# bentherien/point-cloud-reid

Measured on AMD Instinct MI355X. Metric: siamese pair-comparisons/sec @1024 pts, higher is better.
Workload: dtype bf16x3

## Files before the change

point-cloud-reid_amd/csrc/attn_kernels_impl.h:

```cpp
#pragma once
#ifndef PCR_ATTN_PREC
#define PCR_ATTN_PREC 0
#endif
#include "tile_dense.h"

#include <stdio.h>

#include <vector>

namespace {
constexpr int kAPrec = PCR_ATTN_PREC;
struct AttnArgs {
  pcr_attn_params p;
  int dbg;
};

constexpr int kATraceWgs = 512, kATraceRecs = 24, kATraceMarks = 8;
__device__ unsigned long long g_attn_trace[2 * kATraceWgs * kATraceRecs * kATraceMarks];


__device__ __forceinline__ void pos_hidden(float *dst, int RP, const float *P, const float *w0,
                                           const float *b0, int d, int T) {
  for (int e = threadIdx.x; e < d * T; e += blockDim.x) {
    const int o = e / T, t = e - o * T;
    const float v = w0[o * 3] * P[t] + w0[o * 3 + 1] * P[RP + t] + w0[o * 3 + 2] * P[2 * RP + t] + b0[o];
    dst[o * RP + t] = fmaxf(v, 0.f);
  }
}

__device__ __forceinline__ void load_xyz3(float *P, int RP, const float *xyz, int L, int t0, int T) {
  for (int e = threadIdx.x; e < 3 * T; e += blockDim.x) {
    const int c = e / T, t = e - c * T;
    P[c * RP + t] = t0 + t < L ? xyz[(size_t)(t0 + t) * 3 + c] : 0.f;
  }
}

__device__ __forceinline__ void attn_kv_fold_write(const pcr_attn_params &p, const float *KVl, const float *s_kt, size_t b) {
  const int d = p.d, dh = d / p.nhead, ld = d + 1, tid = threadIdx.x;
  float *kv = p.kv + b * ((size_t)d * d + d);
  const int d_o = kThreads / d, d_dd = kThreads - d_o * d;
  int o = tid / d, dd = tid - o * d;
  int v0 = (dd / dh) * dh;
  for (int e = tid; e < d * d; e += kThreads, o += d_o, dd += d_dd) {
    if (dd >= d) {
      dd -= d;
      o++;
    }
    if (d_dd) v0 = (dd / dh) * dh;
    const float *wm = p.wmerge + (size_t)o * d + v0;
    const float *kr = KVl + dd * ld + v0;
    float m = 0.f;
#pragma unroll 8
    for (int v = 0; v < dh; v++) m += wm[v] * kr[v];
    if constexpr (kAPrec == 0) {
      const int kb = dd >> 3, rem = dd & 7;
      kv[(((size_t)kb * d + o) * 2 + (rem & 1)) * 4 + (rem >> 1)] = m;
    } else {
      const int s16 = dd >> 4, kk = dd & 15;
      const int hh = (kk >> 2) & 1, jj = (kk & 3) + ((kk >> 3) << 2);
      const size_t unit = (((size_t)s16 * (d >> 5) + (o >> 5)) * 2) * 64 + hh * 32 + (o & 31);
      const __bf16 hi = (__bf16)m;
      const __bf16 lo = (__bf16)(m - (float)hi);
      __bf16 *img = reinterpret_cast<__bf16 *>(kv);
      img[unit * 8 + jj] = hi;
      img[(unit + 64) * 8 + jj] = lo;
    }
  }
  __syncthreads();
  if (tid < d) kv[(size_t)d * d + tid] = s_kt[tid];
}

__device__ __forceinline__ void attn_kv_fold_mfma(const pcr_attn_params &p, const float *KVt, const float *s_kt, size_t b) {
  const int d = p.d, dh = d / p.nhead, ld = d + 1, tid = threadIdx.x;
  float *kv = p.kv + b * ((size_t)d * d + d);
  for (int hd = 0; hd < p.nhead; hd++) {
    const float *wm = p.wmerge_packed + (size_t)(hd * dh / 8) * d * 8;
    tile_dense(KVt + (size_t)(hd * dh) * ld + hd * dh, dh, ld, dh >> 5, wm, d, [&](float m, int o, int t) {
      const int dd = hd * dh + t;
      if constexpr (kAPrec == 0) {
        const int kb = dd >> 3, rem = dd & 7;
        kv[(((size_t)kb * d + o) * 2 + (rem & 1)) * 4 + (rem >> 1)] = m;
      } else {
        const int s16 = dd >> 4, kk = dd & 15;
        const int hh = (kk >> 2) & 1, jj = (kk & 3) + ((kk >> 3) << 2);
        const size_t unit = (((size_t)s16 * (d >> 5) + (o >> 5)) * 2) * 64 + hh * 32 + (o & 31);
        const __bf16 hi = (__bf16)m;
        const __bf16 lo = (__bf16)(m - (float)hi);
        __bf16 *img = reinterpret_cast<__bf16 *>(kv);
        img[unit * 8 + jj] = hi;
        img[(unit + 64) * 8 + jj] = lo;
      }
    });
  }
  __syncthreads();
  if (tid < d) kv[(size_t)d * d + tid] = s_kt[tid];
}

// ... 1200 lines not shown
          const float tm = up ? vm[r + N] : vm[r], um = up ? vm[r] : vm[r + N];                       \
          const float ts = up ? vs[r + N] : vs[r], us = up ? vs[r] : vs[r + N];                       \
          vm[r] = fmaxf(tm, __uint_as_float(pcr_sort_partner<2 * J, J>(__float_as_uint(um), lane)));  \
          vs[r] = ts + __uint_as_float(pcr_sort_partner<2 * J, J>(__float_as_uint(us), lane));        \
        }                                                                                             \
      }
      PCR_POOL_STEP(8, 2, 2)
      PCR_POOL_STEP(4, 4, 4)
      PCR_POOL_STEP(2, 8, 8)
      PCR_POOL_STEP(1, 16, 16)
#undef PCR_POOL_STEP
      pmax = fmaxf(pmax, vm[0]);
      psum += vs[0];
      if (++pblk == nblk) {
        const int e = ((j & 1) << 4) | ((j & 2) << 2) | (j & 4) | ((j & 8) >> 2) | ((j & 16) >> 4);
        const int ch = 16 * (e >> 3) + bf_kpos(h, e & 7);
        float *po = p.pool_out + (size_t)b * 128;
        po[ch] = pmax;
        po[64 + ch] = psum;
        pmax = -INFINITY;
        psum = 0.f;
        pblk = 0;
        pc += nwav;
      }
    } else if constexpr (!CF) {
      const __amdgpu_buffer_rsrc_t rout =
          __builtin_amdgcn_make_buffer_rsrc(p.out + (size_t)b * (32 * NOB) * p.Lq, 0, 32 * NOB * p.Lq * 4, 0x00020000);
#pragma unroll
      for (int e = 0; e < 16 * NOB; e++) {
        const int ch = 16 * (e >> 3) + bf_kpos(0, e & 7);
        const float v = o[e >> 4][e & 15];
        __builtin_amdgcn_raw_buffer_store_b32(__builtin_bit_cast(unsigned, v), rout, vo, ch * p.Lq * 4, 0);
      }
    } else {
#pragma unroll
      for (int cb = 0; cb < NOB; cb++)
#pragma unroll
        for (int G = 0; G < 2; G++) to_ops(o[cb], G, bh[2 * cb + G], bl[2 * cb + G]);
      f32x16 fo[CF ? CF : 1];
#pragma unroll
      for (int cb = 0; cb < CF; cb++)
#pragma unroll
        for (int r = 0; r < 16; r++) fo[cb][r] = 0.f;
      const bf16x8 *wb = reinterpret_cast<const bf16x8 *>(p.wfinal) + lane;
#pragma unroll
      for (int s2 = 0; s2 < 2 * NOB; s2++) {
        bf16x8 wh[CF ? CF : 1], wl[CF ? CF : 1];
#pragma unroll
        for (int cb = 0; cb < CF; cb++) {
          wh[cb] = wb[((s2 * CF + cb) * 2) * 64];
          wl[cb] = wb[((s2 * CF + cb) * 2 + 1) * 64];
        }
#pragma unroll
        for (int cb = 0; cb < CF; cb++) fo[cb] = __builtin_amdgcn_mfma_f32_32x32x16_bf16(wh[cb], bh[s2], fo[cb], 0, 0, 0);
#pragma unroll
        for (int cb = 0; cb < CF; cb++) fo[cb] = __builtin_amdgcn_mfma_f32_32x32x16_bf16(wh[cb], bl[s2], fo[cb], 0, 0, 0);
#pragma unroll
        for (int cb = 0; cb < CF; cb++) fo[cb] = __builtin_amdgcn_mfma_f32_32x32x16_bf16(wl[cb], bh[s2], fo[cb], 0, 0, 0);
      }
      const __amdgpu_buffer_rsrc_t rout =
          __builtin_amdgcn_make_buffer_rsrc(p.out + (size_t)b * (32 * CF) * p.Lq, 0, 32 * CF * p.Lq * 4, 0x00020000);
#pragma unroll
      for (int cb = 0; cb < CF; cb++)
#pragma unroll
        for (int g = 0; g < 4; g++) {
          const f32x4 bv = cvec(s_c + 320, cb, g);
#pragma unroll
          for (int qq = 0; qq < 4; qq++) {
            const int e = 16 * cb + 4 * g + qq;
            const int ch = 16 * (e >> 3) + bf_kpos(0, e & 7);
            const float v = fo[cb][4 * g + qq] + bv[qq];
            __builtin_amdgcn_raw_buffer_store_b32(__builtin_bit_cast(unsigned, v), rout, vo, ch * p.Lq * 4, 0);
          }
        }
    }
    __builtin_amdgcn_wave_barrier();
    PCR_AMARK(7);
    PCR_ANEXT();
  }
#undef PCR_AMARK
#undef PCR_ANEXT
}

template <int NB>
__device__ __forceinline__ void ap128_step(f32x16 (&acc)[NB], const bf16x8 *wb, int ls, const bf16x8 &bh, const bf16x8 &bl) {
#pragma unroll
  for (int c0 = 0; c0 < NB; c0 += 4) {
    bf16x8 wh[4], wl[4];
#pragma unroll
    for (int cb = 0; cb < 4; cb++) {
      wh[cb] = wb[((ls * NB + c0 + cb) * 2) * 64];
      wl[cb] = wb[((ls * NB + c0 + cb) * 2 + 1) * 64];
    }
#pragma unroll
    for (int cb = 0; cb < 4; cb++) acc[c0 + cb] = __builtin_amdgcn_mfma_f32_32x32x16_bf16(wh[cb], bh, acc[c0 + cb], 0, 0, 0);
#pragma unroll
    for (int cb = 0; cb < 4; cb++) acc[c0 + cb] = __builtin_amdgcn_mfma_f32_32x32x16_bf16(wh[cb], bl, acc[c0 + cb], 0, 0, 0);
#pragma unroll
    for (int cb = 0; cb < 4; cb++) acc[c0 + cb] = __builtin_amdgcn_mfma_f32_32x32x16_bf16(wl[cb], bh, acc[c0 + cb], 0, 0, 0);
    asm volatile("" ::: "memory");
  }
}
constexpr int kAp128Waves = 4, kAp128ChunkU = 2048, kAp128Chunks = 16;
constexpr size_t kAp128Lds = (size_t)2 * kAp128ChunkU * 16 + (640 + 4 * 128 + kAp128Waves * 128) * sizeof(float);
template <int NH>
__global__ __launch_bounds__(64 * kAp128Waves) __attribute__((amdgpu_waves_per_eu(1, 1)))
void attn_apply_stream128_kernel(AttnArgs a) {
  constexpr int D = 128, ND = 4, SD = 8, GPH = 8 / NH;
  constexpr int NPC = kAp128ChunkU / (64 * kAp128Waves);
  extern __shared__ __attribute__((aligned(16))) float smem[];
  const pcr_attn_params &p = a.p;
  f32x4 *s_ring = reinterpret_cast<f32x4 *>(smem);
  int coff = 2 * kAp128ChunkU * 4;
  asm volatile("" : "+s"(coff));
  float *s_c = smem + coff;
  f32x4 *s_p0 = reinterpret_cast<f32x4 *>(s_c + 640);
  float *s_ks = s_c + 640 + 4 * 128;
  const int tid = threadIdx.x, lane = tid & 63, j = lane & 31, h = lane >> 5;
  const int wave = __builtin_amdgcn_readfirstlane(tid >> 6);
  const __amdgpu_buffer_rsrc_t rwq = __builtin_amdgcn_make_buffer_rsrc(const_cast<float *>(p.wq), 0, 4 * kAp128ChunkU * 16, 0x00020000),
                               rw0 = __builtin_amdgcn_make_buffer_rsrc(const_cast<float *>(p.wmlp0), 0, 8 * kAp128ChunkU * 16, 0x00020000),
                               rw2 = __builtin_amdgcn_make_buffer_rsrc(const_cast<float *>(p.wmlp2), 0, 4 * kAp128ChunkU * 16, 0x00020000);
  f32x4 stg[NPC];
  auto fetch = [&](int k) __attribute__((always_inline)) {
    k %= kAp128Chunks;
    const __amdgpu_buffer_rsrc_t r = k < 4 ? rwq : (k < 12 ? rw0 : rw2);
    const int kk = k < 4 ? k : (k < 12 ? k - 4 : k - 12);
#pragma unroll
    for (int u = 0; u < NPC; u++)
      stg[u] = __builtin_bit_cast(f32x4, __builtin_amdgcn_raw_buffer_load_b128(r, tid * 16, (kk * kAp128ChunkU + u * 64 * kAp128Waves) * 16, 0));
    asm volatile("" ::: "memory");
  };
  auto commit = [&](int k) __attribute__((always_inline)) {
    f32x4 *dst = s_ring + (k & 1) * kAp128ChunkU + tid;
#pragma unroll
    for (int u = 0; u < NPC; u++) dst[u * 64 * kAp128Waves] = stg[u];
    __syncthreads();
  };
  for (int e = tid; e < D; e += 64 * kAp128Waves) {
    s_c[e] = p.bq[e];
    s_c[128 + e] = p.ln1_g[e];
    s_c[256 + e] = p.ln1_b[e];
    s_c[384 + e] = p.ln2_g[e];
    s_c[512 + e] = p.ln2_b[e];
    s_p0[e] = f32x4{p.pos0_w[3 * e], p.pos0_w[3 * e + 1], p.pos0_w[3 * e + 2], p.pos0_b[e]};
  }
  fetch(0);
  commit(0);
  const int nblk = p.Lq >> 5;
  const long nitem = (long)p.B * nblk;
  const float skf = (float)p.Sk;
  float *ksw = s_ks + wave * 128;
  auto cvec = [&](const float *base, int cb, int g) __attribute__((always_inline)) {
    return *reinterpret_cast<const f32x4 *>(base + 32 * cb + 8 * g + 4 * h);
  };
  auto to_ops = [&](const f32x16 &acc, int G, bf16x8 &oh, bf16x8 &ol) __attribute__((always_inline)) {
    float v[8];
#pragma unroll
    for (int e = 0; e < 8; e++) v[e] = acc[8 * G + e];
    bf_split8(v, oh, ol, true);
  };
  auto layernorm = [&](f32x16 (&v)[ND], const float *gam, const float *bet) __attribute__((always_inline)) {
    float sm = 0.f;
#pragma unroll
    for (int cb = 0; cb < ND; cb++)
#pragma unroll
      for (int r = 0; r < 16; r++) sm += v[cb][r];
    sm += __shfl_xor(sm, 32, 64);
    const float mean = sm / (float)D;
    float vr = 0.f;
#pragma unroll
    for (int cb = 0; cb < ND; cb++)
#pragma unroll
      for (int r = 0; r < 16; r++) {
        const float dlt = v[cb][r] - mean;
        vr += dlt * dlt;
      }
    vr += __shfl_xor(vr, 32, 64);
    const float inv = 1.0f / sqrtf(vr / (float)D + 1e-5f);
#pragma unroll
    for (int cb = 0; cb < ND; cb++)
#pragma unroll
      for (int g = 0; g < 4; g++) {
        const f32x4 gv = cvec(gam, cb, g), bv = cvec(bet, cb, g);
#pragma unroll
        for (int qq = 0; qq < 4; qq++) v[cb][4 * g + qq] = (v[cb][4 * g + qq] - mean) * inv * gv[qq] + bv[qq];
      }
  };
  for (long it0 = (long)blockIdx.x * kAp128Waves; it0 < nitem; it0 += (long)gridDim.x * kAp128Waves) {
    const long item = it0 + wave;
    const bool live = item < nitem;
    const long it = live ? item : nitem - 1;
    const long b = it / nblk;
    const int blk = (int)(it - b * nblk);
    const size_t bq_ = p.q_index ? (size_t)p.q_index[b] : (size_t)b;
    const size_t kb_ = p.kv_index ? (size_t)p.kv_index[b] : (size_t)b;
    const float *kvp = p.kv + kb_ * ((size_t)D * D + D);
    const int t = blk * 32 + j;
    const __amdgpu_buffer_rsrc_t rfeat = __builtin_amdgcn_make_buffer_rsrc(
        const_cast<float *>(p.feat_q + bq_ * D * p.Lq), 0, D * p.Lq * 4, 0x00020000);
    const int vo = (4 * h * p.Lq + t) * 4;
    auto load_x = [&](float (&xf)[64]) __attribute__((always_inline)) {
#pragma unroll
      for (int e = 0; e < 64; e++) {
        const int ch = 16 * (e >> 3) + bf_kpos(0, e & 7);
        xf[e] = __builtin_bit_cast(float, __builtin_amdgcn_raw_buffer_load_b32(rfeat, vo, ch * p.Lq * 4, 0));
      }
    };
    ksw[lane] = kvp[(size_t)D * D + lane];
    ksw[64 + lane] = kvp[(size_t)D * D + 64 + lane];
    bf16x8 bh[16], bl[16];
    {
      float xf[64];
      load_x(xf);
      const float *xyz = p.xyz_q + (bq_ * p.Lq + t) * 3;
      const float px = xyz[0], py = xyz[1], pz = xyz[2];
#pragma unroll
      for (int s2 = 0; s2 < SD; s2++) {
        float hv[8];
#pragma unroll
        for (int e = 0; e < 8; e++) {
// ... 70 lines not shown
#pragma unroll
        for (int r = 0; r < 16; r++) q[cb][r] = 0.f;
      const bf16x8 *mb = reinterpret_cast<const bf16x8 *>(kvp) + lane;
      bf16x8 mh[2][ND], ml[2][ND];
#pragma unroll
      for (int cb = 0; cb < ND; cb++) {
        mh[0][cb] = mb[(cb * 2) * 64];
        ml[0][cb] = mb[(cb * 2 + 1) * 64];
      }
#pragma unroll
      for (int s2 = 0; s2 < SD; s2++) {
        const int c = s2 & 1;
        if (s2 + 1 < SD) {
#pragma unroll
          for (int cb = 0; cb < ND; cb++) {
            mh[c ^ 1][cb] = mb[(((s2 + 1) * ND + cb) * 2) * 64];
            ml[c ^ 1][cb] = mb[(((s2 + 1) * ND + cb) * 2 + 1) * 64];
          }
        }
        asm volatile("" ::: "memory");
#pragma unroll
        for (int cb = 0; cb < ND; cb++) q[cb] = __builtin_amdgcn_mfma_f32_32x32x16_bf16(mh[c][cb], ch_[s2], q[cb], 0, 0, 0);
#pragma unroll
        for (int cb = 0; cb < ND; cb++) q[cb] = __builtin_amdgcn_mfma_f32_32x32x16_bf16(mh[c][cb], cl_[s2], q[cb], 0, 0, 0);
#pragma unroll
        for (int cb = 0; cb < ND; cb++) q[cb] = __builtin_amdgcn_mfma_f32_32x32x16_bf16(ml[c][cb], ch_[s2], q[cb], 0, 0, 0);
      }
    }
    layernorm(q, s_c + 128, s_c + 256);
#pragma unroll
    for (int cb = 0; cb < ND; cb++)
#pragma unroll
      for (int G = 0; G < 2; G++) to_ops(q[cb], G, bh[SD + 2 * cb + G], bl[SD + 2 * cb + G]);
    f32x16 f[2 * ND];
#pragma unroll
    for (int cb = 0; cb < 2 * ND; cb++)
#pragma unroll
      for (int r = 0; r < 16; r++) f[cb][r] = 0.f;
#pragma unroll
    for (int k = 4; k < 12; k++) {
      fetch(k + 1);
      const bf16x8 *wb = reinterpret_cast<const bf16x8 *>(s_ring + (k & 1) * kAp128ChunkU) + lane;
#pragma unroll
      for (int ls = 0; ls < 2; ls++) ap128_step<2 * ND>(f, wb, ls, bh[2 * (k - 4) + ls], bl[2 * (k - 4) + ls]);
      commit(k + 1);
    }
    float xf[64];
    load_x(xf);
    f32x16 o[ND];
#pragma unroll
    for (int cb = 0; cb < ND; cb++)
#pragma unroll
      for (int r = 0; r < 16; r++) o[cb][r] = 0.f;
#pragma unroll
    for (int k = 12; k < 16; k++) {
      fetch(k + 1);
      bf16x8 oh[4], ol[4];
#pragma unroll
      for (int i = 0; i < 2; i++) {
        f32x16 &fc = f[2 * (k - 12) + i];
#pragma unroll
        for (int r = 0; r < 16; r++) fc[r] = relu_i(fc[r]);
#pragma unroll
        for (int G = 0; G < 2; G++) to_ops(fc, G, oh[2 * i + G], ol[2 * i + G]);
      }
      const bf16x8 *wb = reinterpret_cast<const bf16x8 *>(s_ring + (k & 1) * kAp128ChunkU) + lane;
#pragma unroll
      for (int ls = 0; ls < 4; ls++) ap128_step<ND>(o, wb, ls, oh[ls], ol[ls]);
      commit(k + 1);
    }
    layernorm(o, s_c + 384, s_c + 512);
#pragma unroll
    for (int cb = 0; cb < ND; cb++)
#pragma unroll
      for (int r = 0; r < 16; r++) o[cb][r] += xf[16 * cb + r];
    if (live) {
      const __amdgpu_buffer_rsrc_t rout =
          __builtin_amdgcn_make_buffer_rsrc(p.out + (size_t)b * D * p.Lq, 0, D * p.Lq * 4, 0x00020000);
#pragma unroll
      for (int e = 0; e < 16 * ND; e++) {
        const int ch = 16 * (e >> 3) + bf_kpos(0, e & 7);
        const float v = o[e >> 4][e & 15];
        __builtin_amdgcn_raw_buffer_store_b32(__builtin_bit_cast(unsigned, v), rout, vo, ch * p.Lq * 4, 0);
      }
    }
  }
}
#endif

}

static int attn_check(const pcr_attn_params &p) {
  if (p.B < 0 || p.Lq < 1 || p.Sk < 1 || p.c1 < 1 || p.c2 < 1 || p.cout < 1 || p.nhead < 1) return 1;
  if (p.d < 32 || p.d > 512 || (p.d & 31) || p.d % p.nhead) return 1;
  if (p.d > 128 && ((p.d & 63) || ((p.d / p.nhead) & 63) || p.d / p.nhead > 256)) return 1;
  if ((p.c2 & 7) || p.cout > 512 || p.cfinal > 512) return 1;
  if (!p.feat_q || !p.feat_k || !p.xyz_k || !p.kv || !p.pos0_w || !p.pos0_b || !p.wq || !p.bq || !p.wkv ||
      !p.bkv || !p.wmerge || !p.wmlp0 || !p.wmlp2 || !p.ln1_g || !p.ln1_b || !p.ln2_g || !p.ln2_b)
    return 1;
  if (p.q_pos && (!p.xyz_q || p.c1 != p.c2 || p.c1 != p.d)) return 1;
  if (p.residual && p.cout != p.c1) return 1;
  if (p.cfinal && (!p.wfinal || !p.bfinal || (p.cout & 7))) return 1;
  return 0;
}

static void attn_dump_trace(const char *path, const char *tag, int wgs, int B, int Sk) {
  static int launches = 0;
  static const int skip = pcr_tune_int("PCR_SA_TRACE_SKIP");
  launches++;
  if (launches <= skip || launches > skip + 8) return;
  static std::vector<unsigned long long> host(2 * kATraceWgs * kATraceRecs * kATraceMarks);
  if (hipDeviceSynchronize() != hipSuccess) return;
  if (hipMemcpyFromSymbol(host.data(), HIP_SYMBOL(g_attn_trace), host.size() * sizeof(unsigned long long)) != hipSuccess) return;
  FILE *f = fopen(path, "a");
  if (!f) return;
  const int n = 2 * (wgs < kATraceWgs ? wgs : kATraceWgs);
  fprintf(f, "launch %d kernel %s wgs %d B %d Sk %d\n", launches, tag, wgs, B, Sk);
  for (int w = 0; w < n; w++) {
    const unsigned long long *t = host.data() + (size_t)w * (kATraceRecs * kATraceMarks);
    fprintf(f, "wg %d", w);
    for (int i = 0; i < kATraceRecs * kATraceMarks; i++) fprintf(f, " %llu", t[i]);
    fprintf(f, "\n");
  }
  fclose(f);
}

static int attn_kv_narrow(const pcr_attn_params *pp, pcr_stream_t stream) {
  AttnArgs a;
  a.p = *pp;
  a.dbg = 0;
  const int d = pp->d;
  if (pp->c2 < pp->d) return PCR_ERR_INVALID;
  const int tb = d <= 64 ? 2 : 1, RP = 32 * tb + 1;
  size_t lds = (size_t)(pp->c2 + d + 3) * RP + 4 * d;
  const size_t lds2 = (size_t)d * (d + 1) + d;
  if (lds2 > lds) lds = lds2;
  lds = (lds + kThreads) * sizeof(float);
  if (lds > (size_t)kMaxDynLds) return PCR_ERR_INVALID;
  static bool ok = allow_big_lds(attn_kv_kernel<2, 1, 2, 1>) && allow_big_lds(attn_kv_kernel_o3<2, 1, 1, 1>) &&
                   allow_big_lds(attn_kv_kernel_o3<1, 2, 1, 4>) && allow_big_lds(attn_kv_kernel<1, 2, 0, 4>);
  (void)ok;
  const int ntile = (pp->Sk + 32 * tb - 1) / (32 * tb);
  int ns = pp->kv_splits > 1 ? pp->kv_splits : 1;
  if (ns > 1 && (!pp->kv_part || ns > 64)) return PCR_ERR_INVALID;
  if (ns > ntile) ns = ntile;
  a.p.kv_splits = ns;
  dim3 g(pp->B, ns), blk(kThreads);
  hipStream_t st = pcr_s(stream);
  constexpr bool kBfUnit = kAPrec != 0;
  const bool bfk = kBfUnit && pp->wkv_bf != nullptr;
  if (ns == 1 && d == 64 && (pp->c2 == 64 || (pp->c2 == 128 && bfk && pp->Sk >= 128)) && (pp->Sk & 31) == 0 && pp->nhead >= 1 &&
      64 % pp->nhead == 0) {
    const bool bf = bfk;
    const bool wide = pp->c2 == 128;
    pcr_note_arith(bf ? PCR_PREC_BF16X3 : PCR_PREC_F32);
    static bool oks = allow_big_lds(attn_kv_stream64_kernel<true, false>) && allow_big_lds(attn_kv_stream64_kernel<false, false>) &&
                      allow_big_lds(attn_kv_stream64_kernel<true, kBfUnit>) && allow_big_lds(attn_kv_stream64_kernel<false, kBfUnit>) &&
                      allow_big_lds(attn_kv_stream64_kernel<true, kBfUnit, kBfUnit ? 8 : 4>) &&
                      allow_big_lds(attn_kv_stream64_kernel<false, kBfUnit, kBfUnit ? 8 : 4>);
    (void)oks;
    const int nblk = pp->Sk >> 5;
    const int minw = wide ? 4 : 2;
    int wpc2 = 1;
    while (wpc2 * 2 <= (nblk < 4 ? nblk : 4)) wpc2 *= 2;
    if (wpc2 < minw) wpc2 = minw;
    static const int no_onew = pcr_tune_int("PCR_ATTN_NO_ONEW");
    const bool onew = kBfUnit && bf && !wide && nblk <= 4 && !no_onew;
    if (onew) wpc2 = 1;
    const int cpg = kKvsWaves / wpc2;
    const size_t wu = bf ? (size_t)((wide ? 8 : 4) + 4) * 512 : 4096;
    const size_t lds_s = (wu * 4 + 256 + 128 + 64 * 65 + (onew ? (size_t)0 : (size_t)cpg * (64 * 65 + 64))) * sizeof(float);
    const long rounds = ((long)pp->B + cpg - 1) / cpg;
    static const int ncu = [] {
      hipDeviceProp_t pr;
      int dev = 0;
      if (hipGetDevice(&dev) != hipSuccess || hipGetDeviceProperties(&pr, dev) != hipSuccess) return 256;
      return pr.multiProcessorCount > 0 ? pr.multiProcessorCount : 256;
    }();
    const int gs = (int)(rounds < ncu ? rounds : ncu);
    const dim3 gg(gs), bb(64 * kKvsWaves);
    if (bf && wide) {
      if (pp->nhead >= 2) hipLaunchKernelGGL((attn_kv_stream64_kernel<true, kBfUnit, kBfUnit ? 8 : 4>), gg, bb, lds_s, st, a);
      else hipLaunchKernelGGL((attn_kv_stream64_kernel<false, kBfUnit, kBfUnit ? 8 : 4>), gg, bb, lds_s, st, a);
    } else if (bf) {
      static const char *atrace = pcr_tune_str("PCR_ATTN_TRACE");
      if (atrace) a.dbg |= 256;
      if (onew) {
        static bool oko = allow_big_lds(attn_kv_stream64_kernel<true, kBfUnit, 4, kBfUnit>) &&
                          allow_big_lds(attn_kv_stream64_kernel<false, kBfUnit, 4, kBfUnit>);
        (void)oko;
        if (pp->nhead >= 2) hipLaunchKernelGGL((attn_kv_stream64_kernel<true, kBfUnit, 4, kBfUnit>), gg, bb, lds_s, st, a);
        else hipLaunchKernelGGL((attn_kv_stream64_kernel<false, kBfUnit, 4, kBfUnit>), gg, bb, lds_s, st, a);
      } else if (pp->nhead >= 2) hipLaunchKernelGGL((attn_kv_stream64_kernel<true, kBfUnit>), gg, bb, lds_s, st, a);
      else hipLaunchKernelGGL((attn_kv_stream64_kernel<false, kBfUnit>), gg, bb, lds_s, st, a);
      if (atrace) attn_dump_trace(atrace, "kv64", gs, (int)pp->B, pp->Sk);
    } else {
      if (pp->nhead >= 2) hipLaunchKernelGGL((attn_kv_stream64_kernel<true, false>), gg, bb, lds_s, st, a);
      else hipLaunchKernelGGL((attn_kv_stream64_kernel<false, false>), gg, bb, lds_s, st, a);
    }
    PCR_CHECK_LAUNCH();
    return PCR_OK;
  }
#if PCR_ATTN_PREC != 0
  if (ns == 1 && d == 32 && pp->c2 == 32 && pp->wkv_bf && (pp->Sk & 31) == 0 && pp->nhead >= 1 && 32 % pp->nhead == 0) {
    static bool ok32 = allow_big_lds(attn_kv_stream32_kernel);
    (void)ok32;
    pcr_note_arith(PCR_PREC_BF16X3);
    const int nblk = pp->Sk >> 5;
    int wpc2 = 1;
    while (wpc2 * 2 <= (nblk < kKvsWaves ? nblk : kKvsWaves)) wpc2 *= 2;
    if (wpc2 < 2) wpc2 = 2;
    const int cpg = kKvsWaves / wpc2;
    const size_t lds_s = (size_t)(4096 + 128 + 64 + 32 * 33 + cpg * (32 * 33 + 32)) * sizeof(float);
    const long rounds = ((long)pp->B + cpg - 1) / cpg;
    static const int ncu = [] {
      hipDeviceProp_t pr;
      int dev = 0;
      if (hipGetDevice(&dev) != hipSuccess || hipGetDeviceProperties(&pr, dev) != hipSuccess) return 256;
      return pr.multiProcessorCount > 0 ? pr.multiProcessorCount : 256;
    }();
    const long cap = 2L * ncu;
    hipLaunchKernelGGL(attn_kv_stream32_kernel, dim3((unsigned)(rounds < cap ? rounds : cap)), dim3(64 * kKvsWaves), lds_s, st, a);
    PCR_CHECK_LAUNCH();
    return PCR_OK;
  }
#endif
  pcr_note_arith(PCR_PREC_F32);
  if (d == 32) hipLaunchKernelGGL((attn_kv_kernel<2, 1, 2, 1>), g, blk, lds, st, a);
  else if (d == 64) hipLaunchKernelGGL((attn_kv_kernel_o3<2, 1, 1, 1>), g, blk, lds, st, a);
  else if (d == 128) {
    static bool ok2 = allow_big_lds(attn_kv_kernel_o2<1, 2, 1, 4>) && allow_big_lds(attn_kv_kernel_o2<1, 2, 1, 4, true>);
    (void)ok2;
    if (kBfUnit && pp->wkv_bf && pp->Sk >= 256) hipLaunchKernelGGL((attn_kv_kernel_o2<1, 2, 1, 4, true>), g, blk, lds, st, a);
    else hipLaunchKernelGGL((attn_kv_kernel_o2<1, 2, 1, 4>), g, blk, lds, st, a);
  }
  else hipLaunchKernelGGL((attn_kv_kernel<1, 2, 0, 4>), g, blk, lds, st, a);
  PCR_CHECK_LAUNCH();
  if (ns > 1) {
    static bool okf = allow_big_lds(attn_kv_fold_kernel);
    (void)okf;
    hipLaunchKernelGGL(attn_kv_fold_kernel, dim3(pp->B), blk, ((size_t)d * (d + 1) + d) * sizeof(float), st, a);
    PCR_CHECK_LAUNCH();
  }
  return PCR_OK;
}

static int attn_apply_launch(const pcr_attn_params *pp, pcr_stream_t stream) {
  const pcr_attn_params &p = *pp;
  AttnArgs a;
  a.p = p;
  a.dbg = 0;
  const int tb = p.d <= 32 ? 4 : (p.d <= 64 ? 2 : 1), T = 32 * tb, RP = T + 1;
  const int catP = ceil8(p.c1 + p.d);
  int rowsU = catP > 2 * p.d ? catP : 2 * p.d;
  if (ceil32(p.cout) > rowsU) rowsU = ceil32(p.cout);
  if (ceil32(p.cfinal) > rowsU) rowsU = ceil32(p.cfinal);
  size_t lds = ((size_t)(rowsU + 3 + p.nhead) * RP + 2 * (kThreads / T) * T + 7 * p.d + 2 * p.cout) *
               sizeof(float);
  if (lds > (size_t)kMaxDynLds) return PCR_ERR_INVALID;
  dim3 g((p.Lq + T - 1) / T, p.B), blk(kThreads);
  hipStream_t st = pcr_s(stream);
  pcr_note_arith(kAPrec != 0 ? PCR_PREC_BF16X3 : PCR_PREC_F32);
#if PCR_ATTN_PREC != 0
  const int aps_c1s = (p.c1 + 15) >> 4, aps_nd = p.d >> 5;
  const size_t aps_lds = (size_t)((aps_c1s + (p.q_pos ? 2 * aps_nd : 0)) * aps_nd * 128 + (aps_c1s + 2 * aps_nd) * aps_nd * 256 +
                                  aps_nd * (p.cout >> 5) * 512) * 16 +
                         (size_t)(448 + 256 + 64 * kApsWaves) * sizeof(float);
  static const int no_s128 = pcr_tune_int("PCR_ATTN_NO_STREAM128");
  if (p.d == 128 && p.c1 == 128 && p.cout == 128 && !p.cfinal && p.q_pos && p.residual && (p.Lq & 31) == 0 && p.Lq >= 256 &&
      (p.nhead == 1 || p.nhead == 2 || p.nhead == 4) && !no_s128) {
    const long nitem = (long)p.B * (p.Lq >> 5);
    const long nwg = (nitem + kAp128Waves - 1) / kAp128Waves;
    static const int ncu = [] {
      hipDeviceProp_t pr;
      int dev = 0;
      if (hipGetDevice(&dev) != hipSuccess || hipGetDeviceProperties(&pr, dev) != hipSuccess) return 256;
      return pr.multiProcessorCount > 0 ? pr.multiProcessorCount : 256;
    }();
    const dim3 gg((unsigned)(nwg < ncu ? nwg : ncu)), bb(64 * kAp128Waves);
    static bool ok128 = allow_big_lds(attn_apply_stream128_kernel<1>) && allow_big_lds(attn_apply_stream128_kernel<2>) &&
                        allow_big_lds(attn_apply_stream128_kernel<4>);
    (void)ok128;
    if (p.nhead == 1) hipLaunchKernelGGL((attn_apply_stream128_kernel<1>), gg, bb, kAp128Lds, st, a);
    else if (p.nhead == 2) hipLaunchKernelGGL((attn_apply_stream128_kernel<2>), gg, bb, kAp128Lds, st, a);
    else hipLaunchKernelGGL((attn_apply_stream128_kernel<4>), gg, bb, kAp128Lds, st, a);
    PCR_CHECK_LAUNCH();
    return PCR_OK;
  }
  if (p.d == 32 && p.c1 == 32 && p.cout == 32 && !p.cfinal && (p.Lq & 31) == 0 && (p.nhead == 1 || p.nhead == 2)) {
    const long nitem = (long)p.B * (p.Lq >> 5);
    const long nwg = (nitem + kApsWaves - 1) / kApsWaves;
    static const int ncu = [] {
      hipDeviceProp_t pr;
      int dev = 0;
      if (hipGetDevice(&dev) != hipSuccess || hipGetDeviceProperties(&pr, dev) != hipSuccess) return 256;
      return pr.multiProcessorCount > 0 ? pr.multiProcessorCount : 256;
    }();
    const dim3 gg((unsigned)(nwg < ncu ? nwg : ncu)), bb(64 * kApsWaves);
    static bool ok32 = allow_big_lds(attn_apply_stream64_kernel<true, 2, 0, 1, 1>) && allow_big_lds(attn_apply_stream64_kernel<false, 2, 0, 1, 1>);
    (void)ok32;
    if (p.q_pos) hipLaunchKernelGGL((attn_apply_stream64_kernel<true, 2, 0, 1, 1>), gg, bb, aps_lds, st, a);
    else hipLaunchKernelGGL((attn_apply_stream64_kernel<false, 2, 0, 1, 1>), gg, bb, aps_lds, st, a);
    PCR_CHECK_LAUNCH();
    return PCR_OK;
  }
  const bool aps_in = p.c1 == 64 || ((p.c1 == 32 || (p.c1 < 16 && pp->wmlp0_bf_xpad)) && !p.q_pos && !p.residual);
  const bool aps_out = (p.cout == 64 && (p.cfinal == 0 || p.cfinal == 128) && p.c1 >= 32) ||
                       (p.cout == 128 && !p.cfinal && !p.residual && p.c1 == 64) ||
                       (p.cout == 32 && p.cfinal == 64 && !p.residual && p.c1 < 16);
  if (p.d == 64 && aps_in && aps_out &&
      (p.Lq & 31) == 0 && (p.nhead == 1 || p.nhead == 2 || p.nhead == 4) && aps_lds <= (size_t)kMaxDynLds) {
    const int c1s = aps_c1s, sq = c1s + (p.q_pos ? 4 : 0), s0 = c1s + 4;
    const int nob = p.cout >> 5;
    const size_t lds_s = (size_t)(sq * 256 + s0 * 512 + nob * 1024) * 16 + (size_t)(448 + 256 + 64 * kApsWaves) * sizeof(float);
    const long nitem = (long)p.B * (p.Lq >> 5);
    const long nwg = (nitem + kApsWaves - 1) / kApsWaves;
    static const int ncu = [] {
      hipDeviceProp_t pr;
      int dev = 0;
      if (hipGetDevice(&dev) != hipSuccess || hipGetDeviceProperties(&pr, dev) != hipSuccess) return 256;
      return pr.multiProcessorCount > 0 ? pr.multiProcessorCount : 256;
    }();
    const dim3 gg((unsigned)(nwg < ncu ? nwg : ncu)), bb(64 * kApsWaves);
#define PCR_APS(QP, C1Sv, CFv)                                                            \
  do {                                                                                    \
    static bool oks = allow_big_lds(attn_apply_stream64_kernel<QP, C1Sv, CFv>);           \
    (void)oks;                                                                            \
    hipLaunchKernelGGL((attn_apply_stream64_kernel<QP, C1Sv, CFv>), gg, bb, lds_s, st, a); \
  } while (0)
    const bool cf = p.cfinal != 0;
    static const char *aptrace = pcr_tune_str("PCR_ATTN_TRACE");
    if (aptrace) a.dbg = 256;
    if (pp->pool_out) {
      static bool okp = allow_big_lds(attn_apply_stream64_kernel<false, 4, 0, 2, 2, true>);
// ... 5 lines not shown
      return PCR_OK;
    }
    if (nob == 4) {
      static bool ok4 = allow_big_lds(attn_apply_stream64_kernel<true, 4, 0, 4>) && allow_big_lds(attn_apply_stream64_kernel<false, 4, 0, 4>);
      (void)ok4;
      if (p.q_pos) hipLaunchKernelGGL((attn_apply_stream64_kernel<true, 4, 0, 4>), gg, bb, lds_s, st, a);
      else hipLaunchKernelGGL((attn_apply_stream64_kernel<false, 4, 0, 4>), gg, bb, lds_s, st, a);
    } else if (p.c1 < 16) {
      static bool ok1 = allow_big_lds(attn_apply_stream64_kernel<false, 1, 2, 1>);
      (void)ok1;
      hipLaunchKernelGGL((attn_apply_stream64_kernel<false, 1, 2, 1>), gg, bb, lds_s, st, a);
    } else if (p.c1 == 32) { if (cf) PCR_APS(false, 2, 4); else PCR_APS(false, 2, 0); }
    else if (p.q_pos) { if (cf) PCR_APS(true, 4, 4); else PCR_APS(true, 4, 0); }
    else { if (cf) PCR_APS(false, 4, 4); else PCR_APS(false, 4, 0); }
#undef PCR_APS
    if (aptrace) attn_dump_trace(aptrace, "apply64", (int)gg.x, (int)p.B, p.Lq);
    PCR_CHECK_LAUNCH();
    return PCR_OK;
  }
#endif
  const bool wide = 2 * p.d > 128 || p.cout > 128 || p.cfinal > 128;
#define PCR_APPLY(TBv, NRv)                                                          \
  do {                                                                               \
    static bool ok = allow_big_lds(attn_apply_kernel<TBv, NRv>);                     \
    (void)ok;                                                                        \
    hipLaunchKernelGGL((attn_apply_kernel<TBv, NRv>), g, blk, lds, st, a);           \
  } while (0)
  if (tb == 4) {
    if (wide) PCR_APPLY(4, 2);
    else PCR_APPLY(4, 1);
  } else if (tb == 2) {
    if (wide) PCR_APPLY(2, 2);
    else PCR_APPLY(2, 1);
  } else {
    int widest = 2 * p.d > p.cout ? 2 * p.d : p.cout;
    if (p.cfinal > widest) widest = p.cfinal;
#if PCR_ATTN_PREC == 0
    if (widest > 512) PCR_APPLY(1, 8);
    else if (widest > 256) PCR_APPLY(1, 4);
    else PCR_APPLY(1, 2);
#else
    if (widest > 256) return PCR_ERR_INVALID;
    PCR_APPLY(1, 2);
#endif
  }
#undef PCR_APPLY
  PCR_CHECK_LAUNCH();
  return PCR_OK;
}

#if PCR_ATTN_PREC == 1
int pcr_attn_kv_bf3(const pcr_attn_params *pp, pcr_stream_t stream) { return attn_kv_narrow(pp, stream); }
int pcr_attn_apply_bf3(const pcr_attn_params *pp, pcr_stream_t stream) { return attn_apply_launch(pp, stream); }
#else
int pcr_attn_kv_bf3(const pcr_attn_params *pp, pcr_stream_t stream);
int pcr_attn_apply_bf3(const pcr_attn_params *pp, pcr_stream_t stream);

static bool attn_bf(const pcr_attn_params &p, pcr_attn_params &q) {
  const int widest = 2 * p.d > p.cout ? (2 * p.d > p.cfinal ? 2 * p.d : p.cfinal) : (p.cout > p.cfinal ? p.cout : p.cfinal);
  if (p.precision == 0 || p.d > 128 || widest > 256 || !p.wq_bf || !p.wmlp0_bf || !p.wmlp2_bf ||
      (p.cfinal && !p.wfinal_bf))
    return false;
  q = p;
  q.wq = p.wq_bf; q.wmlp0 = p.wmlp0_bf; q.wmlp2 = p.wmlp2_bf; q.wfinal = p.wfinal_bf;
  return true;
}

PCR_EXPORT int pcr_attn_kv_splits(int B, int Sk, int d) {
  (void)B;
  if (Sk < 1 || d > 64) return 1;
  if ((d == 64 || d == 32) && (Sk & 31) == 0) return 1;
  const int ntile = (Sk + 63) / 64;
  return ntile >= 16 ? 4 : (ntile >= 8 ? 2 : 1);
}

PCR_EXPORT int pcr_attn_kv_f32(const pcr_attn_params *pp, pcr_stream_t stream) {
  if (!pp || attn_check(*pp)) return PCR_ERR_INVALID;
  if (pp->B == 0) return PCR_OK;
  const int d = pp->d;
  if (d > 128) {
    AttnArgs a;
    a.p = *pp;
    a.dbg = 0;
    if (!pp->wkv_wide || !pp->bkv_wide || !pp->wmerge_packed || pp->B > 65535) return PCR_ERR_INVALID;
    pcr_note_arith(PCR_PREC_F32);
    const int dh = d / pp->nhead;
    size_t lds = ((size_t)(pp->c2 + d + 3) * 33 + 4 * d + kThreads) * sizeof(float);
    const size_t lds2 = (size_t)dh * 65 * sizeof(float);
    if (lds2 > lds) lds = lds2;
    if (lds > (size_t)kMaxDynLds) return PCR_ERR_INVALID;
    static bool okw = allow_big_lds(attn_kv_wide_kernel<2>) && allow_big_lds(attn_kv_wide_kernel<3>);
    (void)okw;
    dim3 g(d / 64, pp->B), blk(kThreads);
    if (64 + dh <= 256) hipLaunchKernelGGL((attn_kv_wide_kernel<2>), g, blk, lds, pcr_s(stream), a);
    else hipLaunchKernelGGL((attn_kv_wide_kernel<3>), g, blk, lds, pcr_s(stream), a);
    PCR_CHECK_LAUNCH();
    return PCR_OK;
  }
  pcr_attn_params q;
  if (attn_bf(*pp, q)) return pcr_attn_kv_bf3(&q, stream);
  return attn_kv_narrow(pp, stream);
}

static bool attn_pool_ok(const pcr_attn_params &p) {
  pcr_attn_params q;
  return p.d == 64 && p.c1 == 64 && p.cout == 64 && !p.cfinal && !p.q_pos && (p.Lq & 31) == 0 &&
         (p.nhead == 1 || p.nhead == 2 || p.nhead == 4) && attn_bf(p, q);
}

PCR_EXPORT int pcr_attn_apply_pool_ok(const pcr_attn_params *pp) {
  return (pp && !attn_check(*pp) && attn_pool_ok(*pp)) ? 1 : 0;
}

PCR_EXPORT int pcr_attn_apply_f32(const pcr_attn_params *pp, pcr_stream_t stream) {
  if (!pp || attn_check(*pp) || (!pp->out && !pp->pool_out)) return PCR_ERR_INVALID;
  if (pp->pool_out && !attn_pool_ok(*pp)) return PCR_ERR_INVALID;
  if (pp->B == 0) return PCR_OK;
  if (pp->B > 65535) return PCR_ERR_INVALID;
  pcr_attn_params q;
  if (attn_bf(*pp, q)) return pcr_attn_apply_bf3(&q, stream);
  return attn_apply_launch(pp, stream);
}
#endif
```

Measured before the change: 64700.

## Add persistent streaming KV kernel for d=128 with LDS weight ring

Adds a persistent attn_kv_stream128_kernel for d=128 with 2 or 4 heads. It streams the bf16 KV weights through a double-buffered LDS ring and prefetches the next block's features while the current block runs its MFMAs. Waves are split across key blocks, their partial KV sums are reduced through LDS, and the merge projection is folded in before writing packed bf16 hi/lo output. The grid is capped at the CU count, and ring fetch/commit are factored into shared helpers. This adds a new large code path, LDS reduction barriers and the risk of low occupancy when B is small.

```diff
diff --git a/point-cloud-reid_amd/csrc/attn_kernels_impl.h b/point-cloud-reid_amd/csrc/attn_kernels_impl.h
--- a/point-cloud-reid_amd/csrc/attn_kernels_impl.h
+++ b/point-cloud-reid_amd/csrc/attn_kernels_impl.h
@@ -13,6 +13,7 @@
 struct AttnArgs {
   pcr_attn_params p;
   int dbg;
+  int wpc;
 };
 
 constexpr int kATraceWgs = 512, kATraceRecs = 24, kATraceMarks = 8;
@@ -1379,8 +1380,11 @@
 #undef PCR_ANEXT
 }
 
-template <int NB>
+template <int NB, bool TRANS = false>
 __device__ __forceinline__ void ap128_step(f32x16 (&acc)[NB], const bf16x8 *wb, int ls, const bf16x8 &bh, const bf16x8 &bl) {
+  auto mm = [](const bf16x8 &w, const bf16x8 &x, const f32x16 &c) __attribute__((always_inline)) {
+    return TRANS ? __builtin_amdgcn_mfma_f32_32x32x16_bf16(x, w, c, 0, 0, 0) : __builtin_amdgcn_mfma_f32_32x32x16_bf16(w, x, c, 0, 0, 0);
+  };
 #pragma unroll
   for (int c0 = 0; c0 < NB; c0 += 4) {
     bf16x8 wh[4], wl[4];
@@ -1390,21 +1394,33 @@
       wl[cb] = wb[((ls * NB + c0 + cb) * 2 + 1) * 64];
     }
 #pragma unroll
-    for (int cb = 0; cb < 4; cb++) acc[c0 + cb] = __builtin_amdgcn_mfma_f32_32x32x16_bf16(wh[cb], bh, acc[c0 + cb], 0, 0, 0);
-#pragma unroll
-    for (int cb = 0; cb < 4; cb++) acc[c0 + cb] = __builtin_amdgcn_mfma_f32_32x32x16_bf16(wh[cb], bl, acc[c0 + cb], 0, 0, 0);
-#pragma unroll
-    for (int cb = 0; cb < 4; cb++) acc[c0 + cb] = __builtin_amdgcn_mfma_f32_32x32x16_bf16(wl[cb], bh, acc[c0 + cb], 0, 0, 0);
+    for (int cb = 0; cb < 4; cb++) acc[c0 + cb] = mm(wh[cb], bh, acc[c0 + cb]);
+#pragma unroll
+    for (int cb = 0; cb < 4; cb++) acc[c0 + cb] = mm(wh[cb], bl, acc[c0 + cb]);
+#pragma unroll
+    for (int cb = 0; cb < 4; cb++) acc[c0 + cb] = mm(wl[cb], bh, acc[c0 + cb]);
     asm volatile("" ::: "memory");
   }
 }
 constexpr int kAp128Waves = 4, kAp128ChunkU = 2048, kAp128Chunks = 16;
+constexpr int kAp128Npc = kAp128ChunkU / (64 * kAp128Waves);
+__device__ __forceinline__ void ring128_fetch(f32x4 (&stg)[kAp128Npc], __amdgpu_buffer_rsrc_t r, int kk, int tid) {
+#pragma unroll
+  for (int u = 0; u < kAp128Npc; u++)
+    stg[u] = __builtin_bit_cast(f32x4, __builtin_amdgcn_raw_buffer_load_b128(r, tid * 16, (kk * kAp128ChunkU + u * 64 * kAp128Waves) * 16, 0));
+  asm volatile("" ::: "memory");
+}
+__device__ __forceinline__ void ring128_commit(f32x4 *s_ring, const f32x4 (&stg)[kAp128Npc], int k, int tid) {
+  f32x4 *dst = s_ring + (k & 1) * kAp128ChunkU + tid;
+#pragma unroll
+  for (int u = 0; u < kAp128Npc; u++) dst[u * 64 * kAp128Waves] = stg[u];
+  __syncthreads();
+}
 constexpr size_t kAp128Lds = (size_t)2 * kAp128ChunkU * 16 + (640 + 4 * 128 + kAp128Waves * 128) * sizeof(float);
 template <int NH>
 __global__ __launch_bounds__(64 * kAp128Waves) __attribute__((amdgpu_waves_per_eu(1, 1)))
 void attn_apply_stream128_kernel(AttnArgs a) {
   constexpr int D = 128, ND = 4, SD = 8, GPH = 8 / NH;
-  constexpr int NPC = kAp128ChunkU / (64 * kAp128Waves);
   extern __shared__ __attribute__((aligned(16))) float smem[];
   const pcr_attn_params &p = a.p;
   f32x4 *s_ring = reinterpret_cast<f32x4 *>(smem);
@@ -1418,22 +1434,12 @@
   const __amdgpu_buffer_rsrc_t rwq = __builtin_amdgcn_make_buffer_rsrc(const_cast<float *>(p.wq), 0, 4 * kAp128ChunkU * 16, 0x00020000),
                                rw0 = __builtin_amdgcn_make_buffer_rsrc(const_cast<float *>(p.wmlp0), 0, 8 * kAp128ChunkU * 16, 0x00020000),
                                rw2 = __builtin_amdgcn_make_buffer_rsrc(const_cast<float *>(p.wmlp2), 0, 4 * kAp128ChunkU * 16, 0x00020000);
-  f32x4 stg[NPC];
+  f32x4 stg[kAp128Npc];
   auto fetch = [&](int k) __attribute__((always_inline)) {
     k %= kAp128Chunks;
-    const __amdgpu_buffer_rsrc_t r = k < 4 ? rwq : (k < 12 ? rw0 : rw2);
-    const int kk = k < 4 ? k : (k < 12 ? k - 4 : k - 12);
-#pragma unroll
-    for (int u = 0; u < NPC; u++)
-      stg[u] = __builtin_bit_cast(f32x4, __builtin_amdgcn_raw_buffer_load_b128(r, tid * 16, (kk * kAp128ChunkU + u * 64 * kAp128Waves) * 16, 0));
-    asm volatile("" ::: "memory");
+    ring128_fetch(stg, k < 4 ? rwq : (k < 12 ? rw0 : rw2), k < 4 ? k : (k < 12 ? k - 4 : k - 12), tid);
   };
-  auto commit = [&](int k) __attribute__((always_inline)) {
-    f32x4 *dst = s_ring + (k & 1) * kAp128ChunkU + tid;
-#pragma unroll
-    for (int u = 0; u < NPC; u++) dst[u * 64 * kAp128Waves] = stg[u];
-    __syncthreads();
-  };
+  auto commit = [&](int k) __attribute__((always_inline)) { ring128_commit(s_ring, stg, k, tid); };
   for (int e = tid; e < D; e += 64 * kAp128Waves) {
     s_c[e] = p.bq[e];
     s_c[128 + e] = p.ln1_g[e];
@@ -1670,6 +1676,221 @@
         const int ch = 16 * (e >> 3) + bf_kpos(0, e & 7);
         const float v = o[e >> 4][e & 15];
         __builtin_amdgcn_raw_buffer_store_b32(__builtin_bit_cast(unsigned, v), rout, vo, ch * p.Lq * 4, 0);
+      }
+    }
+  }
+}
+
+__host__ __device__ constexpr int attn_kv128_wpc(int nblk) { return nblk >= 32 ? 4 : (nblk >= 16 ? 2 : 1); }
+constexpr size_t kKv128Lds0 = (size_t)2 * kAp128ChunkU * 16 + 128 * 16 + 256 * 4;
+template <int NH>
+__global__ __launch_bounds__(64 * kAp128Waves) __attribute__((amdgpu_waves_per_eu(1, 1)))
+void attn_kv_stream128_kernel(AttnArgs a) {
+  constexpr int D = 128, SD = 8, TPH = 4 / NH, NKV = NH * TPH * TPH;
+  constexpr int KVU = NKV * 16 + 4;
+  typedef unsigned u32x4 __attribute__((ext_vector_type(4)));
+  extern __shared__ __attribute__((aligned(16))) float smem[];
+  const pcr_attn_params &p = a.p;
+  f32x4 *s_ring = reinterpret_cast<f32x4 *>(smem);
+  int coff = 2 * kAp128ChunkU * 4;
+  asm volatile("" : "+s"(coff));
+  f32x4 *s_p0 = reinterpret_cast<f32x4 *>(smem + coff);
+  float *s_bkv = smem + coff + 4 * D;
+  float *s_red = s_bkv + 2 * D;
+  const int tid = threadIdx.x, lane = tid & 63, j = lane & 31, h = lane >> 5;
+  const int wave = __builtin_amdgcn_readfirstlane(tid >> 6);
+  const __amdgpu_buffer_rsrc_t rw = __builtin_amdgcn_make_buffer_rsrc(const_cast<float *>(p.wkv_bf), 0, 8 * kAp128ChunkU * 16, 0x00020000);
+  f32x4 stg[kAp128Npc];
+  auto fetch = [&](int k) __attribute__((always_inline)) { ring128_fetch(stg, rw, k & 7, tid); };
+  auto commit = [&](int k) __attribute__((always_inline)) { ring128_commit(s_ring, stg, k, tid); };
+  for (int e = tid; e < D; e += 64 * kAp128Waves) s_p0[e] = f32x4{p.pos0_w[3 * e], p.pos0_w[3 * e + 1], p.pos0_w[3 * e + 2], p.pos0_b[e]};
+  for (int e = tid; e < 2 * D; e += 64 * kAp128Waves) s_bkv[e] = p.bkv[e];
+  fetch(0);
+  commit(0);
+  const int Sk = p.Sk, nblk = Sk >> 5;
+  const int wpc = a.wpc, cpg = kAp128Waves / wpc;
+  const int cslot = wave / wpc, wsub = wave - cslot * wpc;
+  const int nper = (nblk + wpc - 1) / wpc;
+  const long cstep = (long)gridDim.x * cpg;
+  const float inv_sk = 1.0f / (float)Sk;
+  float xf[64], pxyz[3];
+  auto issue = [&](long bq, int blk) __attribute__((always_inline)) {
+    const __amdgpu_buffer_rsrc_t rfeat =
+        __builtin_amdgcn_make_buffer_rsrc(const_cast<float *>(p.feat_k + (size_t)bq * D * Sk), 0, D * Sk * 4, 0x00020000);
+    const int t = blk * 32 + j, vo = (4 * h * Sk + t) * 4;
+#pragma unroll
+    for (int e = 0; e < 64; e++) {
+      const int ch = 16 * (e >> 3) + bf_kpos(0, e & 7);
+      xf[e] = __builtin_bit_cast(float, __builtin_amdgcn_raw_buffer_load_b32(rfeat, vo, ch * Sk * 4, 0));
+    }
+    const __amdgpu_buffer_rsrc_t rxyz =
+        __builtin_amdgcn_make_buffer_rsrc(const_cast<float *>(p.xyz_k + (size_t)bq * Sk * 3), 0, Sk * 12, 0x00020000);
+#pragma unroll
+    for (int c = 0; c < 3; c++) pxyz[c] = __builtin_bit_cast(float, __builtin_amdgcn_raw_buffer_load_b32(rxyz, t * 12, c * 4, 0));
+    asm volatile("" ::: "memory");
+  };
+  if ((long)blockIdx.x * cpg + cslot < p.B && wsub < nblk) issue((long)blockIdx.x * cpg + cslot, wsub);
+  for (long c0 = (long)blockIdx.x * cpg; c0 < p.B; c0 += cstep) {
+    const long b = c0 + cslot;
+    const bool live = b < p.B;
+    f32x16 kv[NKV];
+#pragma unroll
+    for (int i = 0; i < NKV; i++)
+#pragma unroll
+      for (int r = 0; r < 16; r++) kv[i][r] = 0.f;
+    float ks[4] = {0.f, 0.f, 0.f, 0.f};
+    for (int it = 0; it < nper; it++) {
+      const int blk = wsub + it * wpc;
+      const bool has = live && blk < nblk;
+      const bool last = it + 1 == nper;
+      const long bn = last ? b + cstep : b;
+      const int blkn = last ? wsub : blk + wpc;
+      const bool hasn = bn < p.B && blkn < nblk;
+      bf16x8 bh[SD], bl[SD];
+      if (has) {
+#pragma unroll
+        for (int s2 = 0; s2 < SD; s2++) {
+          float xv[8];
+#pragma unroll
+          for (int e = 0; e < 8; e++) xv[e] = xf[8 * s2 + e];
+          bf_split8(xv, bh[s2], bl[s2], true);
+        }
+      }
+      f32x16 acc[8];
+#pragma unroll
+      for (int cb = 0; cb < 8; cb++)
+#pragma unroll
+        for (int r = 0; r < 16; r++) acc[cb][r] = 0.f;
+#pragma unroll
+      for (int k = 0; k < 8; k++) {
+        fetch(k + 1);
+        if (has) {
+          const bf16x8 *wb = reinterpret_cast<const bf16x8 *>(s_ring + (k & 1) * kAp128ChunkU) + lane;
+#pragma unroll
+          for (int ls = 0; ls < 2; ls++) {
+            if (k < 4) {
+              ap128_step<8, true>(acc, wb, ls, bh[2 * k + ls], bl[2 * k + ls]);
+            } else {
+              const int s2 = 2 * k + ls - SD;
+              float hv[8];
+#pragma unroll
+              for (int e = 0; e < 8; e++) {
+                const f32x4 w = s_p0[16 * s2 + bf_kpos(0, e) + 4 * h];
+                const float v = w[0] * pxyz[0] + w[1] * pxyz[1] + w[2] * pxyz[2] + w[3];
+                hv[e] = relu_i(v);
+              }
+              bf16x8 hh, hl;
+              bf_split8(hv, hh, hl, true);
+              ap128_step<8, true>(acc, wb, ls, hh, hl);
+            }
+          }
+        }
+        commit(k + 1);
+      }
+      if (hasn) issue(bn, blkn);
+      else {
+#pragma unroll
+        for (int e = 0; e < 64; e++) xf[e] = 0.f;
+        pxyz[0] = pxyz[1] = pxyz[2] = 0.f;
+      }
+      if (has) {
+        float bias[8];
+#pragma unroll
+        for (int cb = 0; cb < 8; cb++) bias[cb] = s_bkv[cb * 32 + j];
+#pragma unroll
+        for (int r = 0; r < 16; r++) {
+#pragma unroll
+          for (int cb = 0; cb < 4; cb++) {
+            acc[cb][r] = elu1(acc[cb][r] + bias[cb]);
+            ks[cb] += acc[cb][r];
+            acc[4 + cb][r] = (acc[4 + cb][r] + bias[4 + cb]) * inv_sk;
+          }
+        }
+#pragma unroll
+        for (int i = 0; i < NKV; i++) {
+          const int hd = i / (TPH * TPH), ib = hd * TPH + (i % (TPH * TPH)) / TPH, jb = hd * TPH + i % TPH;
+#pragma unroll
+          for (int r = 0; r < 16; r++) kv[i] = __builtin_amdgcn_mfma_f32_32x32x2f32(acc[4 + jb][r], acc[ib][r], kv[i], 0, 0, 0);
+        }
+      }
+    }
+#pragma unroll
+    for (int cb = 0; cb < 4; cb++) ks[cb] += __shfl_xor(ks[cb], 32, 64);
+    if (wpc > 1) {
+      int ln = lane;
+      asm volatile("" : "+v"(ln));
+      float *red = s_red + (size_t)cslot * KVU * 64 + ln;
+      for (int round = 0; round < wpc; round++) {
+        if (wsub == round) {
+#pragma unroll
+          for (int i = 0; i < NKV; i++)
+#pragma unroll
+            for (int r = 0; r < 16; r++) {
+              float *dst = red + (i * 16 + r) * 64;
+              *dst = round == 0 ? kv[i][r] : *dst + kv[i][r];
+            }
+#pragma unroll
+          for (int cb = 0; cb < 4; cb++) {
+            float *dst = red + (NKV * 16 + cb) * 64;
+            *dst = round == 0 ? ks[cb] : *dst + ks[cb];
+          }
+        }
+        __syncthreads();
+      }
+#pragma unroll
+      for (int i = 0; i < NKV; i++)
+#pragma unroll
+        for (int r = 0; r < 16; r++) kv[i][r] = red[(i * 16 + r) * 64];
+#pragma unroll
+      for (int cb = 0; cb < 4; cb++) ks[cb] = red[(NKV * 16 + cb) * 64];
+    }
+    if (live) {
+      int ln = lane;
+      asm volatile("" : "+v"(ln));
+      const int j = ln & 31, h = ln >> 5;
+      const __amdgpu_buffer_rsrc_t rkv =
+          __builtin_amdgcn_make_buffer_rsrc(p.kv + (size_t)b * ((size_t)D * D + D), 0, (D * D + D) * 4, 0x00020000);
+      const __amdgpu_buffer_rsrc_t rwm = __builtin_amdgcn_make_buffer_rsrc(const_cast<float *>(p.wmerge), 0, D * D * 4, 0x00020000);
+      for (int ob = wsub; ob < 4; ob += wpc) {
+        const int wrow = ((ob * 32 + j) * D + 4 * h) * 4;
+#pragma unroll
+        for (int hd = 0; hd < NH; hd++) {
+          f32x4 w[TPH][4];
+#pragma unroll
+          for (int jj = 0; jj < TPH; jj++)
+#pragma unroll
+            for (int g = 0; g < 4; g++)
+              w[jj][g] = __builtin_bit_cast(f32x4, __builtin_amdgcn_raw_buffer_load_b128(rwm, wrow, ((hd * TPH + jj) * 32 + 8 * g) * 4, 0));
+#pragma unroll
+          for (int dl = 0; dl < TPH; dl++) {
+            const int db = hd * TPH + dl;
+            f32x16 m;
+#pragma unroll
+            for (int r = 0; r < 16; r++) m[r] = 0.f;
+#pragma unroll
+            for (int jj = 0; jj < TPH; jj++) {
+              const int i = hd * TPH * TPH + dl * TPH + jj;
+#pragma unroll
+              for (int r = 0; r < 16; r++) m = __builtin_amdgcn_mfma_f32_32x32x2f32(kv[i][r], w[jj][r >> 2][r & 3], m, 0, 0, 0);
+            }
+#pragma unroll
+            for (int G = 0; G < 2; G++) {
+              float v[8];
+#pragma unroll
+              for (int e = 0; e < 8; e++) v[e] = m[8 * G + e];
+              bf16x8 hi, lo;
+              bf_split8(v, hi, lo, true);
+              const int unit = (((db * 2 + G) * (D >> 5) + ob) * 2) * 64 + h * 32 + j;
+              __builtin_amdgcn_raw_buffer_store_b128(__builtin_bit_cast(u32x4, hi), rkv, unit * 16, 0, 0);
+              __builtin_amdgcn_raw_buffer_store_b128(__builtin_bit_cast(u32x4, lo), rkv, (unit + 64) * 16, 0, 0);
+            }
+          }
+        }
+      }
+      if (wsub == 0 && h == 0) {
+#pragma unroll
+        for (int cb = 0; cb < 4; cb++)
+          __builtin_amdgcn_raw_buffer_store_b32(__builtin_bit_cast(unsigned, ks[cb]), rkv, (D * D + cb * 32 + j) * 4, 0, 0);
       }
     }
   }
@@ -1717,6 +1938,7 @@
   AttnArgs a;
   a.p = *pp;
   a.dbg = 0;
+  a.wpc = 0;
   const int d = pp->d;
   if (pp->c2 < pp->d) return PCR_ERR_INVALID;
   const int tb = d <= 64 ? 2 : 1, RP = 32 * tb + 1;
@@ -1812,6 +2034,30 @@
     PCR_CHECK_LAUNCH();
     return PCR_OK;
   }
+  static const int no_kv128 = pcr_tune_int("PCR_ATTN_NO_KV128");
+  if (ns == 1 && d == 128 && pp->c2 == 128 && pp->wkv_bf && (pp->Sk & 31) == 0 && pp->Sk >= 256 &&
+      (pp->nhead == 2 || pp->nhead == 4) && !no_kv128) {
+    pcr_note_arith(PCR_PREC_BF16X3);
+    a.wpc = attn_kv128_wpc(pp->Sk >> 5);
+    static const int wpc_t = pcr_tune_int("PCR_ATTN_KV128_WPC");
+    if (wpc_t == 1 || wpc_t == 2 || wpc_t == 4) a.wpc = wpc_t;
+    const int cpg = kAp128Waves / a.wpc;
+    const size_t lds_s = kKv128Lds0 + (a.wpc > 1 ? (size_t)cpg * (16 * (16 / pp->nhead) + 4) * 64 * sizeof(float) : 0);
+    const long nwg = ((long)pp->B + cpg - 1) / cpg;
+    static const int ncu = [] {
+      hipDeviceProp_t pr;
+      int dev = 0;
+      if (hipGetDevice(&dev) != hipSuccess || hipGetDeviceProperties(&pr, dev) != hipSuccess) return 256;
+      return pr.multiProcessorCount > 0 ? pr.multiProcessorCount : 256;
+    }();
+    const dim3 gg((unsigned)(nwg < ncu ? nwg : ncu)), bb(64 * kAp128Waves);
+    static bool ok128 = allow_big_lds(attn_kv_stream128_kernel<2>) && allow_big_lds(attn_kv_stream128_kernel<4>);
+    (void)ok128;
+    if (pp->nhead == 2) hipLaunchKernelGGL((attn_kv_stream128_kernel<2>), gg, bb, lds_s, st, a);
+    else hipLaunchKernelGGL((attn_kv_stream128_kernel<4>), gg, bb, lds_s, st, a);
+    PCR_CHECK_LAUNCH();
+    return PCR_OK;
+  }
 #endif
   pcr_note_arith(PCR_PREC_F32);
   if (d == 32) hipLaunchKernelGGL((attn_kv_kernel<2, 1, 2, 1>), g, blk, lds, st, a);
@@ -1838,6 +2084,7 @@
   AttnArgs a;
   a.p = p;
   a.dbg = 0;
+  a.wpc = 0;
   const int tb = p.d <= 32 ? 4 : (p.d <= 64 ? 2 : 1), T = 32 * tb, RP = T + 1;
   const int catP = ceil8(p.c1 + p.d);
   int rowsU = catP > 2 * p.d ? catP : 2 * p.d;
@@ -2009,6 +2256,7 @@
     AttnArgs a;
     a.p = *pp;
     a.dbg = 0;
+    a.wpc = 0;
     if (!pp->wkv_wide || !pp->bkv_wide || !pp->wmerge_packed || pp->B > 65535) return PCR_ERR_INVALID;
     pcr_note_arith(PCR_PREC_F32);
     const int dh = d / pp->nhead;
```

New measurement: 65850 (median of 6 runs). 1.02x the previous value.
